# ahoop004/f110_gymnasium_ros2_jazzy

Hardware: AMD Instinct MI355X
Metric: env-steps/sec at 65536 parallel envs, 1080-beam lidar; scan L2 vs CPU ref (higher is better)
Workload: dtype f64; 1 GPU; 65536 single-agent envs on one GPU; global_envs=65536, envs_per_gpu=65536, agents=1, beams=1080, map=Spielberg_map, integrator=RK4, scan_noise=True, autoreset=True, parallelism=env-shard x1 (no collectives), streams_per_gpu=2, runner_kind=streams

## Files before the change

f110_gymnasium_ros2_jazzy_amd/csrc/f110_internal.h:

```cpp
#pragma once

#include <hip/hip_runtime.h>
#include <stdint.h>

#include "f110_device.h"

namespace f110 {

constexpr int kCtrSlots = 256;
constexpr int kCtrStride = 16;
constexpr int kRayBlock = 256;
constexpr int kMaxMultiBodies = 64;
constexpr int kMaxChunks = 32;

struct PairGeom;

struct StepArgs {
    MapView map;
    TiledMapView tmap;
    const double *sines, *cosines;
    const double *angles, *beam_cos, *side;
    const double *cs2, *bs2;
    f110_params p;
    const f110_params *pa;
    int32_t E, A, B, theta_dis, integrator, ego, autoreset, mode;
    int32_t reset_f32;
    uint8_t *wcost;
    uint32_t *heavy_list;
    uint32_t *heavy_mask;
    uint32_t *heavy_count;
    int32_t heavy_cap, heavy_T, heavy_build, parity, ray_nch;
    uint32_t *hmask;
    PairGeom *geo;
    int32_t geo_ready;
    int32_t hcheck;
    double fov, eps, max_range, dt, lidar_dist, ttc_thresh, noise_std, inc, beam_incr;
    double side_max;
    uint64_t seed;
    int64_t env_offset;
    double *st;
    double *sb;
    int32_t *scnt;
    double *start;
    double *start_rot;
    int32_t *toggles;
    uint8_t *near_start;
    float *lap_times;
    float *lap_counts;
    double *sim_time;
    uint8_t *pending;
    uint64_t *episode;
    uint64_t *nstep;
    double *ray0;
    BeamRun *runs;
    int32_t *nruns;
    double *scan;
    uint8_t *reset_flag;
    uint8_t *ttc_hit;
    uint64_t *noise_step;
    const double *noise_ext;
    const double *spawn;
    int32_t n_spawn;
    const float *actions;
    const double *actions_f64;
    const double *reset_poses;
    const uint8_t *reset_mask;
    f110_outputs out;
    unsigned long long *ctr;
    double *ptab;
    const double *prange;
    uint64_t pseed;
    int64_t max_steps;
    double stall_speed;
    int32_t stall_steps;
    int32_t *stall;
    uint8_t *truncated;
};

inline float obs_reciprocal(float lmax) {
    if (!(lmax >= 0x1p-30f && lmax <= 0x1p30f)) return 0.0f;
    volatile float l = lmax;
    return 1.0f / l;
}

struct PairGeom {
    double rv[8];
    double phi[4];
    double wc, wh;
    int32_t rng[4];
};

struct RayArgs {
    TiledMapView m;
    const double *sines, *cosines;
    const double *ray0;
    const BeamRun *runs;
    const int32_t *nruns;
    const uint8_t *reset_mask;
    double *scan;
    const double *noise_ext;
    const uint64_t *noise_step;
    unsigned long long *ctr;
    double eps, max_range, noise_std;
    uint64_t seed;
    int64_t env_offset;
    int32_t EA, A, B, theta_dis;
    const double *vel;
    const double *beam_cos, *side;
    double ttc_thresh;
    double side_max;
    uint8_t *ttc_hit;
    float *obs;
    float *scans_f32;
    double *scans_f64;
    int32_t obs_len;
    float lidar_max;
    float obs_rinv;
    int32_t G4;
    uint8_t order[kMaxChunks];
    uint64_t *wtrace;
    uint8_t *wcost;
    const uint32_t *heavy_list;
    const uint32_t *heavy_mask;
    const uint32_t *heavy_count;
    int32_t HB, nch;
    int32_t wpb;
    double fx_cx, fx_cy;
    double fx_lim;
    uint32_t fx_zero;
    double fxp_lo, fxp_hx, fxp_hy;
    int32_t fxp_P;
    double fxs_cx, fxs_cy;
    int32_t count_slots;
    const double *cs2, *bs2;
    const uint32_t *hmask;
    PairGeom *geo;
    int32_t geo_blocks;
    const double *st;
    const f110_params *pa;
    double fov, beam_incr;
};

constexpr double kFxMagic = 6291456.0;
constexpr uint32_t kFxU0 = 0x05600000u;
constexpr uint32_t kFxBand = 4u;
constexpr double kFxpBase = 16777216.0;
constexpr uint32_t kFxpBand = 4u;
constexpr double kFxsBase = 1048576.0;
constexpr double kFxsShift = 0x1p-26;
constexpr uint32_t kFxsBand = 64u;
constexpr int kFxsWaves = 8;
constexpr int kFxsLdsTheta = 2048;

using RayKnobs = f110_ray_knobs;
using RayPlan = f110_ray_plan;
RayPlan plan_ray_launch(const RayKnobs &k, bool masked);

struct FxTable {
    const double *dt;
    int32_t w, P;
    uint32_t oob, zero;
};

struct RayLaunch {
    RayKnobs k;
    FxTable rm, rmp;
    uint8_t chunk_order[kMaxChunks];
    uint64_t *wtrace;
    hipEvent_t gate_wait;
    hipEvent_t gate_record;
};

struct ScanArgs {
    MapView map;
    const double *sines, *cosines;
    int32_t B, theta_dis;
    double fov, eps, max_range, inc;
    const double *poses;
    int64_t M;
    double *scans;
    int32_t *lookups;
    int32_t *hit_rc;
    unsigned long long *ctr;
};

struct GapFollowArgs {
    const float *scans;
    int64_t M, scan_stride, action_stride;
    float *actions;
    int32_t *gaps;
    double angle_min, angle_increment;
    int32_t B;
};

struct TrackView {
    const double *xy;
    const double *s;
    const double *tan;
    const double *nrm;
    const double *mid;
    const double *wR, *wL;
    int32_t n, closed;
    double L;
    const int32_t *cell_start, *cell_items;
    const double *cell_mid;
    int32_t gnx, gny;
    double gx0, gy0, gh;
};

struct RewardArgs {
    TrackView track;
    f110_reward_params p;
    const float *obs;
    int64_t E;
    int32_t obs_len, B;
    f110_reward_state *state;
    const uint8_t *reset_mask;
    double *rewards;
};

constexpr int kEpisodeBlock = 256;
struct EpisodeArgs {
    const double *rewards;
    const uint8_t *terminated, *truncated, *was_reset;
    int64_t E;
    f110_episode_state *state;
    double *last_return;
    int32_t *last_length;
    uint8_t *finished;
    f110_episode_totals *totals;
    EpisodePart *part;
};
inline int64_t episode_blocks(int64_t E) { return (E + kEpisodeBlock - 1) / kEpisodeBlock; }
hipError_t launch_episode_stats(const EpisodeArgs &a, hipStream_t s);

constexpr int kTieCap = 4096;
constexpr int kReplayMaxGrid = 1024;
constexpr int kReplayMaxBatch = 8192;
constexpr int kHistRep = 8;

struct ReplayHdr {
    int64_t length;
    int64_t next;
    uint64_t draws;
    double den;
    int32_t replace;
    int32_t pad0_;
    uint32_t prefix;
    uint32_t kleft;
    uint32_t n_lt, n_tie;
    uint32_t overflow;
    uint32_t pad_;
    uint32_t sel_prefix[4], sel_kleft[4];
};

struct ReplayView {
    ReplayHdr *hdr;
    int64_t capacity;
    int32_t obs_dim, act_dim;
    float *obs, *next_obs, *act, *reward, *done, *prio;
    double *wt;
    uint32_t *keys;
    uint32_t *hist;
    double *den_part;
    uint32_t *part;
    uint64_t *sel;
    uint32_t *tie;
    int64_t *pos;
    double alpha;
    float eps;
    uint64_t seed;
};

struct ReplayRows {
    const float *obs, *next_obs, *act, *reward;
    const double *reward64;
    const float *priority;
    const uint8_t *done;
    int64_t obs_stride, next_stride, act_stride;
    int32_t vec4;
};

struct ReplayBatch {
    float *obs, *next_obs, *act, *reward, *done;
    int32_t vec4;
};

hipError_t launch_replay_add_index(const ReplayView &v, const uint8_t *mask, int mask_skip, const float *priority,
                                   int64_t n, hipStream_t s);
hipError_t launch_replay_add_copy(const ReplayView &v, const ReplayRows &in, int64_t n, hipStream_t s);
hipError_t launch_replay_select(const ReplayView &v, int32_t batch, double beta, int64_t *idx, float *w,
                                bool known_full, hipStream_t s);
hipError_t launch_replay_gather(const ReplayView &v, int32_t batch, const int64_t *idx, const ReplayBatch &out,
                                hipStream_t s);
hipError_t launch_replay_update(const ReplayView &v, const int64_t *idx, const float *val, int64_t n, float add_eps,
                                int32_t from_td, int32_t serial, hipStream_t s);
hipError_t prepare_replay(int32_t max_batch);
int replay_grid(int64_t capacity);

constexpr int kNstepMax = 16;
struct NstepView {
    int64_t n_envs;
    int32_t n, obs_dim, act_dim;
    const double *pw;
    int32_t *len, *head;
    double *ret;
    int32_t *k;
    float *obs, *act;
    int32_t *cnt;
    int32_t *store;
    int64_t *base;
    int32_t *e_slot;
    float *e_reward, *e_done;
};

struct NstepRows {
    const float *obs, *act, *next_obs;
    const double *reward;
    const uint8_t *terminated, *truncated, *was_reset;
    int64_t obs_stride, act_stride, next_stride;
    int32_t vec4;
};

hipError_t launch_nstep_push(const ReplayView &v, const NstepView &w, const NstepRows &in, hipStream_t s);
hipError_t launch_nstep_reset(const NstepView &w, const uint8_t *env_mask, hipStream_t s);

struct AdamArgs {
    float *param, *exp_avg, *exp_avg_sq;
    const float *grad;
    int64_t n;
    double lr, beta1, beta2, eps;
    int64_t *step;
    uint32_t *done;
    float *target;
    float tau;
};
hipError_t launch_adam(const AdamArgs &a, hipStream_t s);

hipError_t launch_env_step(const StepArgs &a, const RayLaunch &r, hipStream_t s,
                           hipEvent_t *ev = nullptr);
hipError_t launch_scan_batch(const ScanArgs &a, hipStream_t s);
hipError_t launch_gap_follow(const GapFollowArgs &a, hipStream_t s);
hipError_t launch_reward(const RewardArgs &a, hipStream_t s);
size_t gap_follow_lds_bytes(int B);
hipError_t launch_dynamics_ks_batch(const double *x, const double *u, double *f, int64_t M, const f110_params &p,
                                    hipStream_t s);
hipError_t launch_collision_batch(const double *v1, const double *v2, int64_t M, uint8_t *out, hipStream_t s);
hipError_t launch_collision_multiple(const double *verts, int64_t M, int32_t N, double *collisions, double *idx,
                                     hipStream_t s);
hipError_t launch_dynamics_batch(const double *x, const double *u, double *f, int64_t M, const f110_params &p,
                                 hipStream_t s);

}
```

f110_gymnasium_ros2_jazzy_amd/csrc/f110_kernels.hip:

```cpp
#include <hip/hip_runtime.h>
#include <hip/hip_ext.h>

#include <algorithm>
#include <cmath>

#include "f110_internal.h"

namespace f110 {

constexpr int kBlock = kRayBlock;

static_assert(sizeof(BeamRun) == 24, "BeamRun layout");

__device__ __forceinline__ uint32_t wave_sum(uint32_t v) {
#pragma unroll
    for (int o = 32; o > 0; o >>= 1) v += __shfl_xor(v, o, 64);
    return v;
}

__device__ __forceinline__ void count_rays(unsigned long long *ctr, uint32_t n, uint32_t rays = 1) {
    uint32_t tot = wave_sum(n);
    uint32_t cnt = wave_sum(n ? rays : 0u);
    if ((threadIdx.x & 63) == 0 && cnt) {
        unsigned long long *slot = ctr + (size_t)(blockIdx.x % kCtrSlots) * kCtrStride;
// ... 768 lines not shown
        if (a.HB && ((ld_const(a.heavy_mask + g) >> grp) & 1u)) return;
    }
    wave_stamp_start(a.wtrace);
    const int lane = (int)threadIdx.x;
    const int B = a.B;
    const int b0 = grp * 64 * N;
    const int e = HANDOFF ? g / a.A : g;
    const bool live = !MASK || ld_const(a.reset_mask + e);

    const BeamRun *R = a.runs + (size_t)g * kMaxSeg;
    const int n = ld_const(a.nruns + g);
    int lo = 0, hi = n - 1;
    while (lo < hi) {
        const int mid = (lo + hi + 1) >> 1;
        if (ld_const(&R[mid].start) <= b0) lo = mid;
        else hi = mid - 1;
    }
    int rs[N];
    double t0[N], dl[N];
    {
        const int s0 = ld_const(&R[lo].start);
        const double u0 = ld_const(&R[lo].t0), w0 = ld_const(&R[lo].delta);
#pragma unroll
        for (int r = 0; r < N; ++r) {
            rs[r] = s0;
            t0[r] = u0;
            dl[r] = w0;
        }
    }
    for (int j = lo + 1; j < n; ++j) {
        const int s2 = ld_const(&R[j].start);
        if (s2 > b0 + 64 * N - 1) break;
        const double tj = ld_const(&R[j].t0), dj = ld_const(&R[j].delta);
#pragma unroll
        for (int r = 0; r < N; ++r)
            if (b0 + 64 * r + lane >= s2) {
                rs[r] = s2;
                t0[r] = tj;
                dl[r] = dj;
            }
    }
    const double x00 = ld_const(a.ray0 + g), y00 = ld_const(a.ray0 + a.EA + g);
    const double d00 = ld_const(a.ray0 + 2 * a.EA + g);
    double x[N], y[N], d[N], tot[N], c[N], sn[N];
    int bc[N];
    bool has[N];
#pragma unroll
    for (int r = 0; r < N; ++r) {
        const int b = b0 + 64 * r + lane;
        has[r] = live && b < B;
        bc[r] = b < B ? b : B - 1;
        int ti = (int)(t0[r] + (double)(bc[r] - rs[r]) * dl[r]);
        if (ti >= a.theta_dis) ti = 0;
        c[r] = a.cosines[ti];
        sn[r] = a.sines[ti];
        x[r] = x00;
        y[r] = y00;
        d[r] = has[r] ? d00 : 0.0;
        tot[r] = d[r];
    }

    const FxLoop L = fx_loop(a);
    const uint32_t zero = a.fx_zero;
    uint32_t zero_v;
    asm volatile("v_mov_b32 %0, %1" : "=v"(zero_v) : "s"(zero));
    const uint32_t P = (uint32_t)a.fxp_P;
    uint32_t lane_iters = 0, iters = 0;
    bool fast_car;
    if (PAD) {
        const double ux = fma(x00, L.ir, L.cxk) - kFxpBase, uy = fma(y00, L.ir, L.cyk) - kFxpBase;
        fast_car = (ux >= a.fxp_lo) & (ux < a.fxp_hx) & (uy >= a.fxp_lo) & (uy < a.fxp_hy);
    } else {
        const double qx = fma(x00, L.ir, L.cxk) - kFxMagic, qy = fma(y00, L.ir, L.cyk) - kFxMagic;
        fast_car = fabs(qx) < a.fx_lim && fabs(qy) < a.fx_lim;
    }
    __builtin_amdgcn_s_waitcnt(0);
    if (fast_car) {
        for (;;) {
            uint64_t m[N], any = 0;
#pragma unroll
            for (int r = 0; r < N; ++r) {
                m[r] = __builtin_amdgcn_ballot_w64(dhi(d[r]) != 0u) & __builtin_amdgcn_ballot_w64(tot[r] <= L.mr);
                any |= m[r];
                lane_iters += (uint32_t)__popcll(m[r]);
            }
            if (!any) break;
            ++iters;
            uint32_t off[N];
#pragma unroll
            for (int r = 0; r < N; ++r) {
                off[r] = zero;
                if (m[r]) {
                    const bool act = (dhi(d[r]) != 0u) & (tot[r] <= L.mr);
                    off[r] = PAD ? fxp_offset(a.m, L, x[r], y[r], d[r], c[r], sn[r], act, m[r], zero_v, P)
                                 : fxn_offset(a.m, L, x[r], y[r], d[r], c[r], sn[r], act, m[r], zero);
                }
            }
#pragma unroll
            for (int r = 0; r < N; ++r) d[r] = fx_load(a.m.dt, off[r]);
#pragma unroll
            for (int r = 0; r < N; ++r) tot[r] += d[r];
        }
    } else {
        uint32_t cnt = 0;
#pragma unroll
        for (int r = 0; r < N; ++r)
            while ((dhi(d[r]) != 0u) & (tot[r] <= L.mr)) {
                if (PAD) {
                    x[r] += d[r] * c[r];
                    y[r] += d[r] * sn[r];
                    d[r] = fx_load(a.m.dt, exact_offset_pad(a.m, x[r], y[r], P));
                    tot[r] += d[r];
                } else {
                    fx_step(a.m, L, x[r], y[r], d[r], tot[r], c[r], sn[r]);
                }
                ++cnt;
            }
        lane_iters = wave_sum(cnt);
        iters = wave_max(cnt);
    }

    const RayArgs &K = *kernarg_rays();
    const double v = ld_const(a.vel + g);
    uint32_t lanes = 0;
    const bool noise_on = K.noise_ext || K.noise_std > 0.0;
    const uint32_t key = noise_key(K.seed, (uint64_t)(K.env_offset + e));
    const uint64_t step = noise_on && !K.noise_ext ? ld_const(K.noise_step + e) : 0;
    float pn[N];
    if (!K.noise_ext && K.noise_std > 0.0) {
        if (N == 2) {
            beam_normal_pair_k(key, step, beam_noise_pair(b0 + lane), pn[0], pn[1]);
        } else {
#pragma unroll
            for (int r = 0; r < N; ++r) pn[r] = beam_normal_k(key, step, bc[r]);
        }
    }
#pragma unroll
    for (int r = 0; r < N; ++r) {
        double nz = 0.0;
        if (K.noise_ext) nz = K.noise_ext[(size_t)e * B + bc[r]];
        else if (K.noise_std > 0.0) nz = K.noise_std * (double)pn[r];
        if (has[r])
            fx_epilogue<HANDOFF>(K, g, e, b0 + 64 * r + lane, tot[r], L.mr, nz, v);
        lanes += (uint32_t)__popcll(__builtin_amdgcn_ballot_w64(has[r]));
    }
    if (lane == 0) {
        if (lanes) {
            unsigned long long *cs = K.ctr + (size_t)(blockIdx.x % kCtrSlots) * kCtrStride;
            atomicAdd(cs, (unsigned long long)(lanes + lane_iters));
            atomicAdd(cs + 1, (unsigned long long)lanes);
            if (K.count_slots) atomicAdd(cs + 2, (unsigned long long)iters * (fast_car ? 64ull * N : 64ull));
        }
        if (K.wcost) {
            const uint32_t mx = lanes ? 1u + iters : 0u;
            K.wcost[(size_t)g * ng + grp] = (uint8_t)(mx < 255u ? mx : 255u);
        }
    }
    wave_stamp_end(kernarg_here().wtrace, (uint32_t)grp, (uint32_t)g);
}

__device__ __forceinline__ double beam_theta(const BeamRun *R, int n, int lo, int b0, int bc) {
    int rs = ld_const(&R[lo].start);
    double t0 = ld_const(&R[lo].t0), dl = ld_const(&R[lo].delta);
    for (int j = lo + 1; j < n; ++j) {
        const int s2 = ld_const(&R[j].start);
        if (s2 > b0 + 63) break;
        if (bc >= s2) {
            rs = s2;
            t0 = ld_const(&R[j].t0);
            dl = ld_const(&R[j].delta);
        }
    }
    return t0 + (double)(bc - rs) * dl;
}


constexpr int kRunsLds = 16;

__device__ __forceinline__ double rfl64(double v) {
    const uint64_t u = (uint64_t)__double_as_longlong(v);
    const uint32_t lo = (uint32_t)__builtin_amdgcn_readfirstlane((int)(uint32_t)u);
    const uint32_t hi = (uint32_t)__builtin_amdgcn_readfirstlane((int)(uint32_t)(u >> 32));
    return __longlong_as_double((long long)(((uint64_t)hi << 32) | lo));
}

__device__ __forceinline__ void run_at(const BeamRun *RL, const BeamRun *RG, int j, int &st, double &t0, double &dl) {
    if (j < kRunsLds) {
        st = __builtin_amdgcn_readfirstlane(RL[j].start);
        t0 = rfl64(RL[j].t0);
        dl = rfl64(RL[j].delta);
    } else {
        st = ld_const(&RG[j].start);
        t0 = ld_const(&RG[j].t0);
        dl = ld_const(&RG[j].delta);
    }
}

__device__ __forceinline__ double beam_theta_l(const BeamRun *RL, const BeamRun *RG, int n, int lo, int b0, int bc) {
    int rs;
    double t0, dl;
    run_at(RL, RG, lo, rs, t0, dl);
    for (int j = lo + 1; j < n; ++j) {
        int s2;
        double u0, u1;
        run_at(RL, RG, j, s2, u0, u1);
        if (s2 > b0 + 63) break;
        if (bc >= s2) {
            rs = s2;
            t0 = u0;
            dl = u1;
        }
    }
    return t0 + (double)(bc - rs) * dl;
}

__device__ __forceinline__ bool lane_in(uint64_t mask) {
    return (uint32_t)(mask >> (threadIdx.x & 63)) & 1u;
}

__device__ __forceinline__ float obs_scan_value_fast(double r, float lmax, float rinv) {
    float v = __builtin_fminf((float)r, lmax);
    v = v < 0.0f ? 0.0f : v;
    const float q = v * rinv;
    float q2 = __builtin_fmaf(__builtin_fmaf(-q, lmax, v), rinv, q);
    const bool ieee = !(v >= 0x1p-60f) | (rinv == 0.0f);
    if (__builtin_amdgcn_ballot_w64(ieee)) {
        asm volatile("" ::: "memory");
        if (ieee) q2 = v / lmax;
    }
    return q2;
}

template <class T>
__device__ __forceinline__ T ld_off(const T *base, uint32_t byte_off) {
    return *reinterpret_cast<const T *>(reinterpret_cast<const char *>(base) + byte_off);
}

__device__ __forceinline__ uint32_t fxs_offset_m(const FxLoop &L, double cx, double cy, double &x, double &y,
                                                 double d, double c, double s, uint64_t m, uint32_t zero_v,
                                                 bool &near) {
    x += d * c;
    y += d * s;
    double tx, ty;
    asm("v_fma_f64 %0, %1, %2, %3" : "=v"(tx) : "v"(x), "v"(L.ir), "s"(cx));
    asm("v_fma_f64 %0, %1, %2, %3" : "=v"(ty) : "v"(y), "v"(L.ir), "s"(cy));
    near = min(dlo(tx), dlo(ty)) < 2u * kFxsBand;
    const uint32_t prow = __umul24(dhi(ty), L.k1);
    uint32_t fast, off;
    asm volatile("v_mad_u32_u24 %0, %1, 8, %2" : "=v"(fast) : "v"(dhi(tx)), "v"(prow));
    const uint64_t ms = ((uint64_t)(uint32_t)__builtin_amdgcn_readfirstlane((uint32_t)(m >> 32)) << 32) |
                        (uint64_t)(uint32_t)__builtin_amdgcn_readfirstlane((uint32_t)m);
    asm("v_cndmask_b32 %0, %1, %2, %3" : "=v"(off) : "v"(zero_v), "v"(fast), "s"(ms));
    return off;
}

__device__ __forceinline__ void pair_geometry(double xi, double yi, double yawi, double xj, double yj, double thj,
                                              double length_i, double width_i, int B, double fov, double incr,
                                              double *rv, double *phi, double &wc, double &wh, int32_t *rng) {
    get_vertices(xj, yj, thj, length_i, width_i, rv);
    double ys, yc;
    cr_sincos(yawi, ys, yc);
    const double ego = atan2(ys, yc);
    int lo = 0, hi = 0;
#pragma unroll
    for (int q = 0; q < 4; ++q) {
        const int k = blocked_vertex_beam(xi, yi, ego, rv[2 * q], rv[2 * q + 1], B, fov, incr, phi[q]);
        lo = (q == 0 || k < lo) ? k : lo;
        hi = (q == 0 || k > hi) ? k : hi;
    }
    double c, h;
    box_beam_window(xi, yi, rv, phi, c, h);
    int r0a, r0b, r1a, r1b;
    window_beam_ranges(yawi, fov, incr, B, c, h, r0a, r0b, r1a, r1b);
    wc = c;
    wh = h;
    rng[0] = r0a > lo ? r0a : lo;
    rng[1] = r0b < hi ? r0b : hi;
    rng[2] = r1a > lo ? r1a : lo;
    rng[3] = r1b < hi ? r1b : hi;
}

__device__ __noinline__ void pair_geometry_ool(double xi, double yi, double yawi, double xj, double yj, double thj,
                                               double length_i, double width_i, int B, double fov, double incr,
                                               double *rv, double *phi, double *wc, double *wh, int32_t *rng) {
    pair_geometry(xi, yi, yawi, xj, yj, thj, length_i, width_i, B, fov, incr, rv, phi, *wc, *wh, rng);
}

__device__ __noinline__ void ray_pair_geometry(const RayArgs &a, int blk) {
    const int A = a.A, EA = a.EA;
    const int NP = A - 1;
    const int pr = blk * 64 + (int)(threadIdx.x & 63);
    if (pr >= EA * NP) return;
    const int g = pr / NP, jj = pr - g * NP;
    const int e = g / A, i = g - e * A;
    const int j = jj < i ? jj : jj + 1;
    const int gj = e * A + j;
    const f110_params &pi = a.pa[i];
    PairGeom &o = a.geo[pr];
    pair_geometry(a.st[g], a.st[EA + g], a.st[(size_t)4 * EA + g], a.st[gj], a.st[EA + gj],
                  a.st[(size_t)4 * EA + gj], pi.length, pi.width, a.B, a.fov, a.beam_incr, o.rv, o.phi, o.wc, o.wh,
                  o.rng);
}

template <bool HANDOFF, bool LDS, bool COUNT>
__global__ void __launch_bounds__(LDS ? 64 * kFxsWaves : 64, 8) k_rays_fxs(RayArgs a) {
    static_assert(!(HANDOFF && LDS), "the LDS table is the single-agent kernel's");
    constexpr int NS = 2;
    constexpr int W = LDS ? kFxsWaves : 1;
    __shared__ double2 cs_lds[LDS ? kFxsLdsTheta : 1];
    __shared__ BeamRun runs_l[W][kRunsLds];
    const int wave = LDS ? __builtin_amdgcn_readfirstlane((int)(threadIdx.x >> 6)) : 0;
    if (LDS) {
        constexpr int kIt = (kFxsLdsTheta + 64 * W - 1) / (64 * W);
        static_assert(!LDS || kIt * 64 * W == kFxsLdsTheta, "the copy's slots cover the LDS table exactly");
        const double2 *src = reinterpret_cast<const double2 *>(a.cs2);
        double2 v[kIt];
#pragma unroll
        for (int i = 0; i < kIt; ++i) {
            const int k = (int)threadIdx.x + i * 64 * W;
            v[i] = src[k < a.theta_dis ? k : a.theta_dis - 1];
        }
#pragma unroll
        for (int i = 0; i < kIt; ++i)
            cs_lds[(int)threadIdx.x + i * 64 * W] = v[i];
        __syncthreads();
    }
    const int item = (int)blockIdx.x * W + wave;
    if (item >= (HANDOFF ? a.geo_blocks : 0) + a.EA * a.G4) return;
    if (HANDOFF && item < a.geo_blocks) {
        ray_pair_geometry(kernarg_here(), item);
        return;
    }
    wave_stamp_start_w(a.wtrace, item);
    const int bid = HANDOFF ? item - a.geo_blocks : item;
    const int wj = bid / a.EA;
    const int g = bid - wj * a.EA;
    const int lane = (int)(threadIdx.x & 63);
    const int B = a.B;
    const int e = HANDOFF ? g / a.A : g;
    const int nch = (B + 63) >> 6;
    const int wstride = a.G4;
    const uint32_t hmask = HANDOFF ? (a.hmask ? ld_const(a.hmask + g) : 0xFFFFFFFFu) : 0u;
    const double *dt = a.m.dt;
    const FxLoop L = fx_loop(a);
    const double rx = ld_const(a.ray0 + g), ry = ld_const(a.ray0 + a.EA + g), rd = ld_const(a.ray0 + 2 * a.EA + g);
    const int nr = ld_const(a.nruns + g);
    const BeamRun *RG = a.runs + (size_t)g * kMaxSeg;
    BeamRun *RL = runs_l[wave];
    if (lane < kRunsLds) RL[lane] = RG[lane];
    double x00, y00, d00;
    asm volatile("v_mov_b64 %0, %1" : "=v"(x00) : "s"(rx));
    asm volatile("v_mov_b64 %0, %1" : "=v"(y00) : "s"(ry));
    asm volatile("v_mov_b64 %0, %1" : "=v"(d00) : "s"(rd));
    asm volatile("" ::"s"(nr));
    uint32_t zero_v;
    asm volatile("v_mov_b32 %0, %1" : "=v"(zero_v) : "s"(a.fx_zero));

    double x[NS], y[NS], d[NS], tot[NS], c[NS], sn[NS];
    int kk[NS];
    int kpar[NS];
    int pnext = wj;
    int kinfo = 0;
    uint32_t srch = 0;
    if (nr <= kRunsLds) {
        int cnt = 0;
#pragma unroll
        for (int j = 1; j < kRunsLds; ++j) cnt += (j < nr && RL[j].start <= lane * 64) ? 1 : 0;
        kinfo = cnt;
    } else if (lane < nch) {
        int lo = 0, hi = nr - 1;
        {
            while (lo < hi) {
                const int mid = (lo + hi + 1) >> 1;
                if (RG[mid].start <= lane * 64) lo = mid;
                else hi = mid - 1;
                if (COUNT) ++srch;
            }
        }
        kinfo = lo;
    }
    uint32_t loads = (LDS ? (uint32_t)((a.theta_dis - 64 * wave + 64 * W - 1) / (64 * W)) : 0u) + 2u;
    uint32_t trips = 0;
    auto arm = [&](int r, bool in_loop) {
        const RayArgs &K = kernarg_here();
        const int k = nch - 1 - pnext;
        kpar[r] = (k >> 1) & 1;
        pnext += wstride;
        kk[r] = k;
        const int b = k * 64 + lane, bc = b < B ? b : B - 1;
        const int lo = __builtin_amdgcn_readlane(kinfo, k);
        int ti = (int)beam_theta_l(runs_l[wave], K.runs + (size_t)g * kMaxSeg, ld_const(K.nruns + g), lo, k * 64,
                                   bc);
        if (ti >= K.theta_dis) ti = 0;
        double2 t2;
        if (LDS) {
            t2 = cs_lds[ti];
        } else {
            t2 = ld_off(reinterpret_cast<const double2 *>(K.cs2), (uint32_t)ti * 16u);
            if (COUNT) loads = __builtin_amdgcn_readfirstlane(loads + 1u);
        }
        c[r] = t2.x;
        sn[r] = t2.y;
        x[r] = x00;
        y[r] = y00;
        d[r] = b < B ? d00 : 0.0;
        tot[r] = in_loop ? 0.0 : d[r];
    };
    uint32_t lanes = 0;
    float cval[2] = {0.0f, 0.0f};
    int ctag[2] = {-1, -1};
    auto finish = [&](int r) {
        const RayArgs &K = kernarg_here();
        const int b = kk[r] * 64 + lane;
        const bool inb = b < B;
        const int bc = inb ? b : B - 1;
        double nz = 0.0;
        if (K.noise_ext) {
            nz = K.noise_ext[(size_t)e * B + bc];
            if (COUNT) loads = __builtin_amdgcn_readfirstlane(loads + 1u);
        } else if (K.noise_std > 0.0) {
            const int pp = kk[r] >> 1, ci = kpar[r];
            float nv;
            if (ctag[ci] == pp) {
                nv = cval[ci];
                ctag[ci] = -1;
            } else {
                const uint32_t key = noise_key(K.seed, (uint64_t)(K.env_offset + e));
                float lo, hi;
                beam_normal_pair_k(key, ld_const(K.noise_step + e), beam_noise_pair(b), lo, hi);
                nv = (kk[r] & 1) ? hi : lo;
                cval[ci] = (kk[r] & 1) ? lo : hi;
                ctag[ci] = pp;
            }
            nz = K.noise_std * (double)nv;
        }
        if (inb) {
            const double mr = K.max_range;
            double range = tot[r] > mr ? mr : tot[r];
            if (K.noise_ext || K.noise_std > 0.0) range += nz;
            const double v = ld_const(K.vel + g);
            const uint32_t boff = (uint32_t)bc * 8u;
            if (v != 0.0) {
                const bool may = ttc_may_fire_lane(range, K.side_max, v, K.ttc_thresh);
                if (__builtin_amdgcn_ballot_w64(may)) {
                    const double2 t2 = ld_off(reinterpret_cast<const double2 *>(K.bs2), boff * 2u);
                    if (COUNT) loads = __builtin_amdgcn_readfirstlane(loads + 1u);
                    if (may && ttc_fires(range, t2.x, v * t2.y, K.ttc_thresh)) K.ttc_hit[g] = 1;
                }
            }
            if (K.obs && (!HANDOFF || g == e * K.A)) {
                float *orow = K.obs + (size_t)e * K.obs_len;
                *reinterpret_cast<float *>(reinterpret_cast<char *>(orow) + (uint32_t)b * 4u) =
                    obs_scan_value_fast(range, K.lidar_max, K.obs_rinv);
            }
            const size_t row = (size_t)g * B;
            if (K.scans_f32) *reinterpret_cast<float *>(reinterpret_cast<char *>(K.scans_f32 + row) + (uint32_t)b * 4u) = (float)range;
            if (K.scans_f64) *reinterpret_cast<double *>(reinterpret_cast<char *>(K.scans_f64 + row) + (uint32_t)b * 8u) = range;
            if (HANDOFF && ((hmask >> kk[r]) & 1u))
                *reinterpret_cast<double *>(reinterpret_cast<char *>(K.scan + row) + (uint32_t)b * 8u) = range;
        }
        if (COUNT) lanes += (uint32_t)min(64, B - kk[r] * 64);
    };

    uint32_t lane_iters = 0, slot_gathers = 0;
    uint32_t closed_trips = 0;
    const double ux = fma(ld_const(a.ray0 + g), L.ir, L.cxk) - kFxpBase;
    const double uy = fma(ld_const(a.ray0 + a.EA + g), L.ir, L.cyk) - kFxpBase;
    const bool fast_car = (ux >= a.fxp_lo) & (ux < a.fxp_hx) & (uy >= a.fxp_lo) & (uy < a.fxp_hy);
    if (fast_car) {
#pragma unroll
        for (int r = 0; r < NS; ++r) {
            kk[r] = -1;
            d[r] = tot[r] = x[r] = y[r] = c[r] = sn[r] = 0.0;
        }
#pragma unroll
        for (int r = 0; r < NS; ++r)
            if (pnext < nch) arm(r, true);
        __builtin_amdgcn_s_waitcnt(0);
        uint64_t nb[NS];
        auto slot_step = [&](int r) {
            tot[r] += d[r];
            uint64_t m = __builtin_amdgcn_ballot_w64(dhi(d[r]) != 0u) & __builtin_amdgcn_ballot_w64(tot[r] <= L.mr);
            if (!m && kk[r] >= 0) {
                finish(r);
                if (pnext < nch) {
                    arm(r, false);
                    m = __builtin_amdgcn_ballot_w64(dhi(d[r]) != 0u) & __builtin_amdgcn_ballot_w64(tot[r] <= L.mr);
                } else {
                    kk[r] = -1;
                }
                __builtin_amdgcn_s_waitcnt(0);
            }
            if (COUNT) {
                lane_iters += (uint32_t)__popcll(m);
                ++slot_gathers;
            }
            bool near;
            const uint32_t off = fxs_offset_m(L, a.fxs_cx, a.fxs_cy, x[r], y[r], d[r], c[r], sn[r], m, zero_v, near);
            d[r] = ld_off(dt, off);
            nb[r] = __builtin_amdgcn_ballot_w64(near) & m;
            __builtin_amdgcn_sched_barrier(0);
        };
        auto regather = [&](int r) {
            const RayArgs &K = kernarg_here();
            if (lane_in(nb[r])) d[r] = ld_off(dt, exact_offset_pad(K.m, x[r], y[r], (uint32_t)K.fxp_P));
            if (COUNT) loads = __builtin_amdgcn_readfirstlane(loads + 1u);
        };
        if (kk[1] >= 0) {
            for (;;) {
#pragma unroll
                for (int r = 0; r < NS; ++r) slot_step(r);
                if (nb[0] | nb[1]) {
                    if (nb[0]) regather(0);
                    if (nb[1]) regather(1);
                    __builtin_amdgcn_s_waitcnt(0);
                }
                if (COUNT) ++trips;
                if ((kk[0] < 0) | (kk[1] < 0)) break;
            }
            if (kk[0] < 0) {
                x[0] = x[1];
                y[0] = y[1];
                d[0] = d[1];
                tot[0] = tot[1];
                c[0] = c[1];
                sn[0] = sn[1];
                kk[0] = kk[1];
                kpar[0] = kpar[1];
            }
        }
        while (kk[0] >= 0) {
            slot_step(0);
            if (nb[0]) regather(0);
            if (COUNT) {
                ++trips;
                ++closed_trips;
            }
        }
    } else {
        uint32_t cnt = 0;
        while (pnext < nch) {
            arm(0, false);
            const RayArgs &K = kernarg_here();
            uint32_t cc = 0;
            while ((dhi(d[0]) != 0u) & (tot[0] <= L.mr)) {
                x[0] += d[0] * c[0];
                y[0] += d[0] * sn[0];
                d[0] = ld_off(dt, exact_offset_pad(K.m, x[0], y[0], (uint32_t)K.fxp_P));
                tot[0] += d[0];
                ++cc;
            }
            cnt += cc;
            if (COUNT) trips += wave_max(cc);
            finish(0);
        }
        if (COUNT) {
            lane_iters = wave_sum(cnt);
            slot_gathers = trips;
        }
    }
    if (COUNT) {
        if (lane == 0) {
            const RayArgs &K = kernarg_here();
            unsigned long long *cs = K.ctr + (size_t)(item % kCtrSlots) * kCtrStride;
            atomicAdd(cs, (unsigned long long)(lanes + lane_iters));
            atomicAdd(cs + 1, (unsigned long long)lanes);
            atomicAdd(cs + 2, (unsigned long long)slot_gathers * 64ull);
            atomicAdd(cs + 3, (unsigned long long)loads);
            atomicAdd(cs + 5, (unsigned long long)closed_trips);
        }
        const uint32_t ws = wave_max(srch);
        if (lane == 0) atomicAdd(a.ctr + (size_t)(item % kCtrSlots) * kCtrStride + 3, (unsigned long long)ws);
    }
    wave_stamp_end_w(a.wtrace, item, (uint32_t)(trips < 0xffffu ? trips : 0xffffu) << 8 | (uint32_t)wj, (uint32_t)g);
}

struct EpiCar {
    double sx, sy;
    int32_t tg;
    float lt;
    uint32_t ns;
};
struct EpiEnv {
    double tprev, ct, st;
    uint64_t nstep;
    uint32_t episode;
    int32_t stall;
};


__device__ __forceinline__ void epilogue_load_car(const StepArgs &a, int g, EpiCar &c) {
    const int EA = a.E * a.A;
    c.sx = a.start[g];
    c.sy = a.start[EA + g];
    c.tg = a.toggles[g];
    c.ns = a.near_start[g];
    c.lt = a.lap_times[g];
}

template <bool LIM>
__device__ __forceinline__ void epilogue_load_env(const StepArgs &a, int e, EpiEnv &v) {
    v.tprev = a.sim_time[e];
    v.ct = a.start_rot[e];
    v.st = a.start_rot[a.E + e];
    v.nstep = a.noise_step[e];
    const uint32_t ep = a.episode[e];
    v.episode = a.mode == 0 ? ep : 0u;
    v.stall = (LIM && a.stall_steps) ? a.stall[e] : 0;
}

template <bool LIM>
__device__ void env_epilogue(const StepArgs &a, int e, const double *stl, int stride, const int32_t *col,
                             int do_reset, const EpiEnv &v, const EpiCar *cars, double vego) {
    const int A = a.A;
    const double tnow = (do_reset ? 0.0 : v.tprev) + a.dt;
    a.sim_time[e] = tnow;
    const double r00 = v.ct, r01 = -v.st, r10 = v.st, r11 = v.ct;
    bool all4 = true;
    for (int i = 0; i < A; ++i) {
        const int g = e * A + i;
        const EpiCar &c = cars[i];
        double px = stl[i * stride] - c.sx;
        double py = stl[i * stride + 1] - c.sy;
        double dx = fma(r01, py, r00 * px);
        double dy = fma(r11, py, r10 * px);
        double ty;
        if (dy > 2.0) ty = dy - 2.0;
        else if (dy < -2.0) ty = -2.0 - dy;
        else ty = 0.0;
        bool close = dx * dx + ty * ty <= 0.1;
        int tg = c.tg;
        uint32_t ns = c.ns;
        if (close && !ns) { ns = 1; ++tg; }
        else if (!close && ns) { ns = 0; ++tg; }
        a.toggles[g] = tg;
        a.near_start[g] = (uint8_t)ns;
        float lc = (float)(tg / 2);
        float lt = tg < 4 ? (float)tnow : c.lt;
        a.lap_counts[g] = lc;
        a.lap_times[g] = lt;
        if (a.out.lap_counts) a.out.lap_counts[g] = lc;
        if (a.out.lap_times) a.out.lap_times[g] = lt;
        all4 = all4 && tg >= 4;
    }
    bool term = col[a.ego] || all4;
    if (a.out.terminated) a.out.terminated[e] = term ? 1 : 0;
    if (a.out.was_reset) a.out.was_reset[e] = (uint8_t)do_reset;
    if (a.out.sim_time) a.out.sim_time[e] = tnow;
    bool trunc = false;
    if (LIM) {
        int32_t s = 0;
        if (a.stall_steps) {
            s = do_reset ? 0 : (fabs(vego) < a.stall_speed ? (v.stall < INT32_MAX ? v.stall + 1 : v.stall) : 0);
            a.stall[e] = s;
        }
        const uint8_t code = (term || do_reset) ? (uint8_t)0 : truncation_code(v.nstep, s, a.max_steps, a.stall_steps);
        if (a.truncated) a.truncated[e] = code;
        trunc = code != 0;
    }
    a.pending[e] = (a.autoreset && (term || trunc)) ? 1 : 0;
    const uint32_t ep = do_reset ? (a.mode == 0 ? v.episode + 1 : 0u) : v.episode;
    if (do_reset) a.episode[e] = ep;
    a.nstep[e] = v.nstep + 1;
}

template <bool LIM>
__global__ void __launch_bounds__(64) k_post_single(StepArgs a) {
    reset_next_heavy(a);
    const int e = blockIdx.x * 64 + threadIdx.x;
    if (e >= a.E) return;
    if (a.mode == 1 && a.reset_mask && !a.reset_mask[e]) return;
    const int EA = a.E;
    double stl[2] = {a.st[e], a.st[EA + e]};
    double yaw = a.st[(size_t)4 * EA + e];
    int32_t col = a.ttc_hit[e];
    const int do_reset = a.reset_flag[e];
    const double vego = (LIM && a.stall_steps) ? a.st[(size_t)3 * EA + e] : 0.0;
    EpiCar car;
    EpiEnv env;
    epilogue_load_car(a, e, car);
    epilogue_load_env<LIM>(a, e, env);
    if (col) {
#pragma unroll
        for (int k = 3; k < 7; ++k) a.st[(size_t)k * EA + e] = 0.0;
        yaw = 0.0;
    }
    if (a.out.obs) {
        float *o = a.out.obs + (size_t)e * obs_row(a) + a.B;
        const float4 v = make_float4((float)stl[0], (float)stl[1], (float)wrap_angle(yaw), col ? 1.0f : 0.0f);
        if ((reinterpret_cast<uintptr_t>(o) & 15u) == 0) {
            *reinterpret_cast<float4 *>(o) = v;
        } else {
            o[0] = v.x;
            o[1] = v.y;
            o[2] = v.z;
            o[3] = v.w;
        }
    }
    if (a.out.collisions) a.out.collisions[e] = (uint8_t)col;
    env_epilogue<LIM>(a, e, stl, 2, &col, do_reset, env, &car, col ? 0.0 : vego);
}

__device__ __forceinline__ void wave_sync() {
    __builtin_amdgcn_fence(__ATOMIC_RELEASE, "wavefront");
    __builtin_amdgcn_wave_barrier();
    __builtin_amdgcn_fence(__ATOMIC_ACQUIRE, "wavefront");
}

constexpr int kMultiBlock = 128;

struct MultiShared {
    double stl[kMaxAgents][7];
    double pose0[kMaxAgents][3];
    double verts[kMaxAgents][8];
    double rv[kMaxAgents * (kMaxAgents - 1)][8];
    double wcen[kMaxAgents * (kMaxAgents - 1)], whalf[kMaxAgents * (kMaxAgents - 1)];
    double phi[kMaxAgents * (kMaxAgents - 1)][4];
    double ego[kMaxAgents];
    int32_t kq[kMaxAgents * (kMaxAgents - 1)][4];
    int32_t blo[kMaxAgents * (kMaxAgents - 1)], bhi[kMaxAgents * (kMaxAgents - 1)];
    int32_t rng[kMaxAgents * (kMaxAgents - 1)][4];
    int32_t col[kMaxAgents];
    int32_t ttc[kMaxAgents];
    EpiCar epi[kMaxAgents];
    EpiEnv epe;
    int32_t do_reset;
};

__device__ __forceinline__ int pass_beams(const MultiShared &sh, int pr) {
    const int n0 = sh.rng[pr][1] - sh.rng[pr][0] + 1;
    const int n1 = sh.rng[pr][3] - sh.rng[pr][2] + 1;
    return (n0 > 0 ? n0 : 0) + (n1 > 0 ? n1 : 0);
}


template <bool LIM>
__global__ void __launch_bounds__(kMultiBlock, 6) k_post_multi(StepArgs a) {
    reset_next_heavy(a);
    __shared__ MultiShared sh;
    const int e = blockIdx.x;
    const int tid = threadIdx.x;
    const int A = a.A, B = a.B;
    const int EA = a.E * A;
    if (a.mode == 1 && a.reset_mask && !a.reset_mask[e]) return;
#ifdef F110_POST_PHASES
    uint64_t tph = wall_clock64();
    auto phase = [&](int k) {
        const uint64_t t = wall_clock64();
        if (tid == 0) atomicAdd(a.ctr + (size_t)(e % kCtrSlots) * kCtrStride + 8 + k, (unsigned long long)(t - tph));
        tph = t;
    };
#else
    auto phase = [](int) {};
#endif
    double *scan = a.scan + (size_t)e * A * B;
    if (tid < A) {
        const int g = e * A + tid;
#pragma unroll
        for (int k = 0; k < 7; ++k) sh.stl[tid][k] = a.st[(size_t)k * EA + g];
        sh.pose0[tid][0] = sh.stl[tid][0];
        sh.pose0[tid][1] = sh.stl[tid][1];
        sh.pose0[tid][2] = sh.stl[tid][4];
        epilogue_load_car(a, g, sh.epi[tid]);
        get_vertices(sh.stl[tid][0], sh.stl[tid][1], sh.stl[tid][4], a.p.length, a.p.width, sh.verts[tid]);
        const int hit = a.ttc_hit[g];
        sh.col[tid] = hit;
        sh.ttc[tid] = hit;
        if (hit) {
#pragma unroll
            for (int k = 3; k < 7; ++k) {
                sh.stl[tid][k] = 0.0;
                a.st[(size_t)k * EA + g] = 0.0;
            }
        }
    }
    if (tid == 0) {
        sh.do_reset = a.reset_flag[e];
        epilogue_load_env<LIM>(a, e, sh.epe);
    }
    __syncthreads();
    phase(0);
    if (tid == 0) {
        for (int i = 0; i < A - 1; ++i)
            for (int j = i + 1; j < A; ++j)
                if (gjk_collision(sh.verts[i], sh.verts[j])) {
                    sh.col[i] = 1;
                    sh.col[j] = 1;
                }
    }
    if (tid >= 64 && a.geo_ready) {
        const int lane = tid & 63;
        const int NP = A * (A - 1);
        for (int pr = lane; pr < NP; pr += 64) {
            const int i = pr / (A - 1);
            const int jj = pr - i * (A - 1);
            const int j = jj < i ? jj : jj + 1;
            if (sh.ttc[i]) {
                pair_geometry_ool(sh.stl[i][0], sh.stl[i][1], sh.stl[i][4], sh.pose0[j][0], sh.pose0[j][1],
                                  sh.pose0[j][2], a.pa[i].length, a.pa[i].width, B, a.fov, a.beam_incr, sh.rv[pr],
                                  sh.phi[pr], &sh.wcen[pr], &sh.whalf[pr], sh.rng[pr]);
            } else {
                const PairGeom &o = a.geo[(size_t)e * NP + pr];
#pragma unroll
                for (int k = 0; k < 8; ++k) sh.rv[pr][k] = o.rv[k];
                sh.wcen[pr] = o.wc;
                sh.whalf[pr] = o.wh;
#pragma unroll
                for (int k = 0; k < 4; ++k) sh.rng[pr][k] = o.rng[k];
            }
        }
    } else if (tid >= 64) {
        const int lane = tid & 63;
        const int NP = A * (A - 1);
        for (int pr = lane; pr < NP; pr += 64) {
            const int i = pr / (A - 1);
            const int jj = pr - i * (A - 1);
            const int j = jj < i ? jj : jj + 1;
            const f110_params &pi = a.pa[i];
            get_vertices(sh.pose0[j][0], sh.pose0[j][1], sh.pose0[j][2], pi.length, pi.width, sh.rv[pr]);
        }
        if (lane < A) {
            double ys, yc;
            cr_sincos(sh.stl[lane][4], ys, yc);
            sh.ego[lane] = atan2(ys, yc);
        }
        wave_sync();
        for (int w = lane; w < 4 * NP; w += 64) {
            const int pr = w >> 2, q = w & 3;
            const int i = pr / (A - 1);
            sh.kq[pr][q] = blocked_vertex_beam(sh.stl[i][0], sh.stl[i][1], sh.ego[i], sh.rv[pr][2 * q],
                                               sh.rv[pr][2 * q + 1], B, a.fov, a.beam_incr, sh.phi[pr][q]);
        }
        wave_sync();
        for (int pr = lane; pr < NP; pr += 64) {
            const int i = pr / (A - 1);
            int lo = sh.kq[pr][0], hi = sh.kq[pr][0];
#pragma unroll
            for (int q = 1; q < 4; ++q) {
                lo = sh.kq[pr][q] < lo ? sh.kq[pr][q] : lo;
                hi = sh.kq[pr][q] > hi ? sh.kq[pr][q] : hi;
            }
            sh.blo[pr] = lo;
            sh.bhi[pr] = hi;
            double wc, wh;
            box_beam_window(sh.stl[i][0], sh.stl[i][1], sh.rv[pr], sh.phi[pr], wc, wh);
            sh.wcen[pr] = wc;
            sh.whalf[pr] = wh;
            int r0a, r0b, r1a, r1b;
            window_beam_ranges(sh.stl[i][4], a.fov, a.beam_incr, B, wc, wh, r0a, r0b, r1a, r1b);
            sh.rng[pr][0] = r0a > lo ? r0a : lo;
            sh.rng[pr][1] = r0b < hi ? r0b : hi;
            sh.rng[pr][2] = r1a > lo ? r1a : lo;
            sh.rng[pr][3] = r1b < hi ? r1b : hi;
        }
    }
    __syncthreads();
    phase(1);
    for (int jj = 0; jj < A - 1; ++jj) {
        int total = 0;
        for (int i = 0; i < A; ++i) total += pass_beams(sh, i * (A - 1) + jj);
        for (int item = tid; item < total; item += kMultiBlock) {
            int i = 0, k = item;
            for (int n = pass_beams(sh, jj); k >= n; n = pass_beams(sh, i * (A - 1) + jj)) {
                k -= n;
                ++i;
            }
            const int pr = i * (A - 1) + jj;
            const int n0 = sh.rng[pr][1] - sh.rng[pr][0] + 1;
            const int b = k < (n0 > 0 ? n0 : 0) ? sh.rng[pr][0] + k : sh.rng[pr][2] + k - (n0 > 0 ? n0 : 0);
            const double ox = sh.stl[i][0], oy = sh.stl[i][1], oth = sh.stl[i][4];
            const double *v = sh.rv[pr];
            const double ang = beam_angle(b, a.fov, a.beam_incr);
            if (!(fabs(wrap_pm_pi(oth + ang - sh.wcen[pr])) <= sh.whalf[pr])) continue;
            if ((a.hcheck & 1) && a.hmask && !((a.hmask[(size_t)e * A + i] >> (b >> 6)) & 1u))
                atomicAdd(a.ctr + (size_t)(e % kCtrSlots) * kCtrStride + 6, 1ull);
            const double bt = oth + ang + kPi / 2.;
            double v31, v30;
// ... 353 lines not shown
```

Measured before the change: 102.4 million env-steps/s.

## Hoist per-wave lidar constants to SGPRs and buffer obs stores off the hot loop

In the single-agent lidar kernel, per-env constants (velocity, noise step, noise key, output flags, obs row pointer) are loaded once per wave and held in scalar registers. Scalar kernarg fields are also regrouped into one aligned block so they can be fetched together. Obs scan stores are buffered in a small register ring and flushed in batches, and the full s_waitcnt(0) after each beam finish is replaced with a vmem-only drain. The goal is to cut kernarg reloads and memory-wait stalls in the per-chunk finish path. The cost is extra register pressure and more code complexity, plus optional phase-timing instrumentation.

```diff
diff --git a/f110_gymnasium_ros2_jazzy_amd/csrc/f110_internal.h b/f110_gymnasium_ros2_jazzy_amd/csrc/f110_internal.h
--- a/f110_gymnasium_ros2_jazzy_amd/csrc/f110_internal.h
+++ b/f110_gymnasium_ros2_jazzy_amd/csrc/f110_internal.h
@@ -91,6 +91,14 @@
 };
 
 struct RayArgs {
+    alignas(64) double max_range;
+    double noise_std;
+    double side_max;
+    double ttc_thresh;
+    float lidar_max;
+    float obs_rinv;
+    int32_t theta_dis;
+    int32_t obs_len;
     TiledMapView m;
     const double *sines, *cosines;
     const double *ray0;
@@ -101,21 +109,16 @@
     const double *noise_ext;
     const uint64_t *noise_step;
     unsigned long long *ctr;
-    double eps, max_range, noise_std;
+    double eps;
     uint64_t seed;
     int64_t env_offset;
-    int32_t EA, A, B, theta_dis;
+    int32_t EA, A, B;
     const double *vel;
     const double *beam_cos, *side;
-    double ttc_thresh;
-    double side_max;
     uint8_t *ttc_hit;
     float *obs;
     float *scans_f32;
     double *scans_f64;
-    int32_t obs_len;
-    float lidar_max;
-    float obs_rinv;
     int32_t G4;
     uint8_t order[kMaxChunks];
     uint64_t *wtrace;
diff --git a/f110_gymnasium_ros2_jazzy_amd/csrc/f110_kernels.hip b/f110_gymnasium_ros2_jazzy_amd/csrc/f110_kernels.hip
--- a/f110_gymnasium_ros2_jazzy_amd/csrc/f110_kernels.hip
+++ b/f110_gymnasium_ros2_jazzy_amd/csrc/f110_kernels.hip
@@ -1094,10 +1094,41 @@
                   o.rng);
 }
 
+constexpr uint32_t kFxsNoiseExt = 1u, kFxsNoiseDev = 2u, kFxsObs = 4u, kFxsFull = 8u;
+constexpr int kFxsObsBuf = 4;
+
+#ifdef F110_RAYS_PHASES
+#define RAYS_PHASE_T0() const uint64_t ph_t0 = __builtin_amdgcn_s_memtime()
+#define RAYS_PHASE_T1() ph_pass += __builtin_amdgcn_s_memtime() - ph_t0
+#else
+#define RAYS_PHASE_T0() ((void)0)
+#define RAYS_PHASE_T1() ((void)0)
+#endif
+
+struct FxsPass {
+    double max_range, noise_std, side_max, ttc_thresh;
+    float lidar_max, obs_rinv;
+    int32_t theta_dis;
+};
+
+__device__ __forceinline__ FxsPass fxs_pass(const RayArgs &K) {
+    const FxsPass P{K.max_range, K.noise_std, K.side_max, K.ttc_thresh, K.lidar_max, K.obs_rinv, K.theta_dis};
+    asm volatile("" ::"s"(P.max_range), "s"(P.noise_std), "s"(P.side_max), "s"(P.ttc_thresh), "s"(P.lidar_max),
+                 "s"(P.obs_rinv), "s"(P.theta_dis));
+    return P;
+}
+
+__device__ __forceinline__ void drain_vmem() {
+    __builtin_amdgcn_s_waitcnt(0x0F70);
+}
+
 template <bool HANDOFF, bool LDS, bool COUNT>
 __global__ void __launch_bounds__(LDS ? 64 * kFxsWaves : 64, 8) k_rays_fxs(RayArgs a) {
     static_assert(!(HANDOFF && LDS), "the LDS table is the single-agent kernel's");
     constexpr int NS = 2;
+    constexpr bool HOLD = !HANDOFF;
+    constexpr int D = (LDS && !COUNT) ? kFxsObsBuf : 0;
+    constexpr bool PASS_DRAIN = D == 0;
     constexpr int W = LDS ? kFxsWaves : 1;
     __shared__ double2 cs_lds[LDS ? kFxsLdsTheta : 1];
     __shared__ BeamRun runs_l[W][kRunsLds];
@@ -1124,6 +1155,10 @@
         return;
     }
     wave_stamp_start_w(a.wtrace, item);
+#ifdef F110_RAYS_PHASES
+    const uint64_t ph_start = __builtin_amdgcn_s_memtime();
+    uint64_t ph_pass = 0;
+#endif
     const int bid = HANDOFF ? item - a.geo_blocks : item;
     const int wj = bid / a.EA;
     const int g = bid - wj * a.EA;
@@ -1138,6 +1173,17 @@
     const double rx = ld_const(a.ray0 + g), ry = ld_const(a.ray0 + a.EA + g), rd = ld_const(a.ray0 + 2 * a.EA + g);
     const int nr = ld_const(a.nruns + g);
     const BeamRun *RG = a.runs + (size_t)g * kMaxSeg;
+    const double vel_s = HOLD ? ld_const(a.vel + g) : 0.0;
+    const uint64_t nstep_s = HOLD ? ld_const(a.noise_step + e) : 0ull;
+    uint32_t nkey_s = 0u, flags = 0u;
+    float *orow = nullptr;
+    if (HOLD) {
+        const uint32_t f = (a.noise_ext ? kFxsNoiseExt : a.noise_std > 0.0 ? kFxsNoiseDev : 0u) |
+                           (a.obs ? kFxsObs : 0u) | ((a.scans_f32 || a.scans_f64) ? kFxsFull : 0u);
+        asm volatile("s_mov_b32 %0, %1" : "=s"(flags) : "s"(f));
+        asm volatile("s_mov_b32 %0, %1" : "=s"(nkey_s) : "s"(noise_key(a.seed, (uint64_t)(a.env_offset + e))));
+        orow = a.obs + (size_t)e * a.obs_len;
+    }
     BeamRun *RL = runs_l[wave];
     if (lane < kRunsLds) RL[lane] = RG[lane];
     double x00, y00, d00;
@@ -1145,6 +1191,7 @@
     asm volatile("v_mov_b64 %0, %1" : "=v"(y00) : "s"(ry));
     asm volatile("v_mov_b64 %0, %1" : "=v"(d00) : "s"(rd));
     asm volatile("" ::"s"(nr));
+    if (HOLD) asm volatile("" ::"s"(vel_s), "s"(nstep_s));
     uint32_t zero_v;
     asm volatile("v_mov_b32 %0, %1" : "=v"(zero_v) : "s"(a.fx_zero));
 
@@ -1173,7 +1220,7 @@
     }
     uint32_t loads = (LDS ? (uint32_t)((a.theta_dis - 64 * wave + 64 * W - 1) / (64 * W)) : 0u) + 2u;
     uint32_t trips = 0;
-    auto arm = [&](int r, bool in_loop) {
+    auto arm = [&](int r, bool in_loop, int theta_dis) {
         const RayArgs &K = kernarg_here();
         const int k = nch - 1 - pnext;
         kpar[r] = (k >> 1) & 1;
@@ -1181,9 +1228,9 @@
         kk[r] = k;
         const int b = k * 64 + lane, bc = b < B ? b : B - 1;
         const int lo = __builtin_amdgcn_readlane(kinfo, k);
-        int ti = (int)beam_theta_l(runs_l[wave], K.runs + (size_t)g * kMaxSeg, ld_const(K.nruns + g), lo, k * 64,
-                                   bc);
-        if (ti >= K.theta_dis) ti = 0;
+        int ti = (int)beam_theta_l(runs_l[wave], HOLD ? RG : K.runs + (size_t)g * kMaxSeg,
+                                   HOLD ? nr : ld_const(K.nruns + g), lo, k * 64, bc);
+        if (ti >= theta_dis) ti = 0;
         double2 t2;
         if (LDS) {
             t2 = cs_lds[ti];
@@ -1201,55 +1248,100 @@
     uint32_t lanes = 0;
     float cval[2] = {0.0f, 0.0f};
     int ctag[2] = {-1, -1};
-    auto finish = [&](int r) {
+    float obuf[D > 0 ? D : 1] = {};
+    uint32_t oids = 0u;
+    int nbuf = 0;
+    auto flush = [&](bool in_pass) {
+#pragma unroll
+        for (int j = 0; j < D; ++j) {
+            if (j < nbuf) {
+                const int b = (int)((oids >> (8 * j)) & 255u) * 64 + lane;
+                if (b < B) *reinterpret_cast<float *>(reinterpret_cast<char *>(orow) + (uint32_t)b * 4u) = obuf[j];
+            }
+        }
+        nbuf = 0;
+        if (in_pass && !PASS_DRAIN) drain_vmem();
+    };
+    auto finish = [&](int r, const FxsPass &P) {
         const RayArgs &K = kernarg_here();
         const int b = kk[r] * 64 + lane;
         const bool inb = b < B;
         const int bc = inb ? b : B - 1;
+        uint32_t fl = 0u, nkey = 0u;
+        if (HOLD) {
+            asm volatile("s_mov_b32 %0, %1" : "=s"(fl) : "s"(flags));
+            asm volatile("s_mov_b32 %0, %1" : "=s"(nkey) : "s"(nkey_s));
+        }
+        const bool ext = HOLD ? (fl & kFxsNoiseExt) != 0u : K.noise_ext != nullptr;
+        const double nstd = HOLD ? P.noise_std : K.noise_std;
+        const bool dev = HOLD ? (fl & kFxsNoiseDev) != 0u : (!ext && nstd > 0.0);
+        const bool now = D == 0 || (fl & kFxsFull) != 0u;
         double nz = 0.0;
-        if (K.noise_ext) {
+        if (ext) {
             nz = K.noise_ext[(size_t)e * B + bc];
             if (COUNT) loads = __builtin_amdgcn_readfirstlane(loads + 1u);
-        } else if (K.noise_std > 0.0) {
+            if (!PASS_DRAIN) drain_vmem();
+        } else if (dev) {
             const int pp = kk[r] >> 1, ci = kpar[r];
             float nv;
             if (ctag[ci] == pp) {
                 nv = cval[ci];
                 ctag[ci] = -1;
             } else {
-                const uint32_t key = noise_key(K.seed, (uint64_t)(K.env_offset + e));
+                const uint32_t key = HOLD ? nkey : noise_key(K.seed, (uint64_t)(K.env_offset + e));
                 float lo, hi;
-                beam_normal_pair_k(key, ld_const(K.noise_step + e), beam_noise_pair(b), lo, hi);
+                beam_normal_pair_k(key, HOLD ? nstep_s : ld_const(K.noise_step + e), beam_noise_pair(b), lo, hi);
                 nv = (kk[r] & 1) ? hi : lo;
                 cval[ci] = (kk[r] & 1) ? lo : hi;
                 ctag[ci] = pp;
             }
-            nz = K.noise_std * (double)nv;
-        }
+            nz = nstd * (double)nv;
+        }
+        float oval = 0.0f;
         if (inb) {
-            const double mr = K.max_range;
+            const double mr = HOLD ? P.max_range : K.max_range;
             double range = tot[r] > mr ? mr : tot[r];
-            if (K.noise_ext || K.noise_std > 0.0) range += nz;
-            const double v = ld_const(K.vel + g);
+            if (ext || dev) range += nz;
+            const double v = HOLD ? vel_s : ld_const(K.vel + g);
             const uint32_t boff = (uint32_t)bc * 8u;
             if (v != 0.0) {
-                const bool may = ttc_may_fire_lane(range, K.side_max, v, K.ttc_thresh);
+                const double thr = HOLD ? P.ttc_thresh : K.ttc_thresh;
+                const bool may = ttc_may_fire_lane(range, HOLD ? P.side_max : K.side_max, v, thr);
                 if (__builtin_amdgcn_ballot_w64(may)) {
                     const double2 t2 = ld_off(reinterpret_cast<const double2 *>(K.bs2), boff * 2u);
                     if (COUNT) loads = __builtin_amdgcn_readfirstlane(loads + 1u);
-                    if (may && ttc_fires(range, t2.x, v * t2.y, K.ttc_thresh)) K.ttc_hit[g] = 1;
+                    if (may && ttc_fires(range, t2.x, v * t2.y, thr)) K.ttc_hit[g] = 1;
+                    if (!PASS_DRAIN) drain_vmem();
                 }
             }
-            if (K.obs && (!HANDOFF || g == e * K.A)) {
-                float *orow = K.obs + (size_t)e * K.obs_len;
-                *reinterpret_cast<float *>(reinterpret_cast<char *>(orow) + (uint32_t)b * 4u) =
-                    obs_scan_value_fast(range, K.lidar_max, K.obs_rinv);
+            const float lmax = HOLD ? P.lidar_max : K.lidar_max, rinv = HOLD ? P.obs_rinv : K.obs_rinv;
+            if (HOLD ? (fl & kFxsObs) != 0u : (K.obs && g == e * K.A)) {
+                const float ov = obs_scan_value_fast(range, lmax, rinv);
+                if (now) {
+                    float *row = HOLD ? orow : K.obs + (size_t)e * K.obs_len;
+                    *reinterpret_cast<float *>(reinterpret_cast<char *>(row) + (uint32_t)b * 4u) = ov;
+                } else {
+                    oval = ov;
+                }
             }
             const size_t row = (size_t)g * B;
-            if (K.scans_f32) *reinterpret_cast<float *>(reinterpret_cast<char *>(K.scans_f32 + row) + (uint32_t)b * 4u) = (float)range;
-            if (K.scans_f64) *reinterpret_cast<double *>(reinterpret_cast<char *>(K.scans_f64 + row) + (uint32_t)b * 8u) = range;
+            if (!HOLD || (fl & kFxsFull)) {
+                if (K.scans_f32) *reinterpret_cast<float *>(reinterpret_cast<char *>(K.scans_f32 + row) + (uint32_t)b * 4u) = (float)range;
+                if (K.scans_f64) *reinterpret_cast<double *>(reinterpret_cast<char *>(K.scans_f64 + row) + (uint32_t)b * 8u) = range;
+            }
             if (HANDOFF && ((hmask >> kk[r]) & 1u))
                 *reinterpret_cast<double *>(reinterpret_cast<char *>(K.scan + row) + (uint32_t)b * 8u) = range;
+        }
+        if (D > 0) {
+            if (now) {
+                if (!PASS_DRAIN) drain_vmem();
+            } else if (fl & kFxsObs) {
+#pragma unroll
+                for (int j = D - 1; j > 0; --j) obuf[j] = obuf[j - 1];
+                obuf[0] = oval;
+                oids = (oids << 8) | (uint32_t)kk[r];
+                if (++nbuf == D) flush(true);
+            }
         }
         if (COUNT) lanes += (uint32_t)min(64, B - kk[r] * 64);
     };
@@ -1267,21 +1359,26 @@
         }
 #pragma unroll
         for (int r = 0; r < NS; ++r)
-            if (pnext < nch) arm(r, true);
+            if (pnext < nch) arm(r, true, a.theta_dis);
         __builtin_amdgcn_s_waitcnt(0);
         uint64_t nb[NS];
         auto slot_step = [&](int r) {
             tot[r] += d[r];
             uint64_t m = __builtin_amdgcn_ballot_w64(dhi(d[r]) != 0u) & __builtin_amdgcn_ballot_w64(tot[r] <= L.mr);
             if (!m && kk[r] >= 0) {
-                finish(r);
+                RAYS_PHASE_T0();
+                const RayArgs &K = kernarg_here();
+                FxsPass P{};
+                if (HOLD) P = fxs_pass(K);
+                finish(r, P);
                 if (pnext < nch) {
-                    arm(r, false);
+                    arm(r, false, HOLD ? P.theta_dis : K.theta_dis);
                     m = __builtin_amdgcn_ballot_w64(dhi(d[r]) != 0u) & __builtin_amdgcn_ballot_w64(tot[r] <= L.mr);
                 } else {
                     kk[r] = -1;
                 }
-                __builtin_amdgcn_s_waitcnt(0);
+                if (PASS_DRAIN) __builtin_amdgcn_s_waitcnt(0);
+                RAYS_PHASE_T1();
             }
             if (COUNT) {
                 lane_iters += (uint32_t)__popcll(m);
@@ -1332,8 +1429,10 @@
     } else {
         uint32_t cnt = 0;
         while (pnext < nch) {
-            arm(0, false);
             const RayArgs &K = kernarg_here();
+            FxsPass P{};
+            if (HOLD) P = fxs_pass(K);
+            arm(0, false, HOLD ? P.theta_dis : K.theta_dis);
             uint32_t cc = 0;
             while ((dhi(d[0]) != 0u) & (tot[0] <= L.mr)) {
                 x[0] += d[0] * c[0];
@@ -1344,12 +1443,17 @@
             }
             cnt += cc;
             if (COUNT) trips += wave_max(cc);
-            finish(0);
+            finish(0, P);
         }
         if (COUNT) {
             lane_iters = wave_sum(cnt);
             slot_gathers = trips;
         }
+    }
+    if (D > 0 && nbuf) {
+        RAYS_PHASE_T0();
+        flush(false);
+        RAYS_PHASE_T1();
     }
     if (COUNT) {
         if (lane == 0) {
@@ -1365,6 +1469,12 @@
         if (lane == 0) atomicAdd(a.ctr + (size_t)(item % kCtrSlots) * kCtrStride + 3, (unsigned long long)ws);
     }
     wave_stamp_end_w(a.wtrace, item, (uint32_t)(trips < 0xffffu ? trips : 0xffffu) << 8 | (uint32_t)wj, (uint32_t)g);
+#ifdef F110_RAYS_PHASES
+    if (a.wtrace && lane == 0) {
+        const uint64_t whole = __builtin_amdgcn_s_memtime() - ph_start;
+        a.wtrace[4 * (size_t)item + 2] = (ph_pass << 32) | (whole & 0xffffffffull);
+    }
+#endif
 }
 
 struct EpiCar {
```

Result: no change. 103.3 million env-steps/s, median of 6 (+0.9%).
